# tohinz/multiple-objects-gan

Hardware: AMD Instinct MI355X
Metric: images/sec per G+D train step, 256x256 coco-attngan (higher is better)
Workload: dtype f32

## Files before the change

### include/mogan_hip.h

```cpp
#ifndef MOGAN_HIP_H
#define MOGAN_HIP_H

#include <stddef.h>
#include <stdint.h>

#ifdef __cplusplus
extern "C" {
#endif

typedef struct ihipStream_t* hipStream_t;

#define MOGAN_ERR_SHAPE (-1)
#define MOGAN_ERR_LAUNCH (-2)
#define MOGAN_ERR_WS (-3)

#define MOGAN_ACT_NONE 0
#define MOGAN_ACT_RELU 1
#define MOGAN_ACT_LRELU 2
#define MOGAN_ACT_GLU 3
#define MOGAN_ACT_TANH 4
#define MOGAN_ACT_SIGMOID 5

int mogan_abi_version(void);
int mogan_gemm_set_split_target(int blocks);
// ... 59 lines not shown
                          const int* dgrad, hipStream_t stream);
int mogan_conv2d_fwd_wp(const float* x, const float* w, const void* wprep, float* y, int B, int Cin, int Hs, int Ws, int Cout, int KH,
                        int KW, int stride, int ph, int pw, int up, void* ws, size_t ws_bytes, hipStream_t stream);
int mogan_conv2d_dgrad_wp(const float* dy, const float* w, const void* wprep, float* dx, int B, int Cin, int Hs, int Ws, int Cout,
                          int KH, int KW, int stride, int ph, int pw, int up, void* ws, size_t ws_bytes, hipStream_t stream);
int mogan_conv2d_wgrad(const float* dy, const float* x, float* dw, int B, int Cin, int Hs, int Ws, int Cout, int KH,
                       int KW, int stride, int ph, int pw, int up, int accumulate, void* ws, size_t ws_bytes,
                       hipStream_t stream);

int mogan_pk_conv_eligible(int B, int Cin, int Hs, int Ws, int Cout, int KH, int KW, int stride, int ph, int pw, int dgrad);
size_t mogan_pk_weight_bytes(int Cout, int Cin, int KH, int KW, int stride, int dgrad);
int mogan_pk_weight_pack(const float* w, void* wpk, int Cout, int Cin, int KH, int KW, int stride, int ph, int pw, int dgrad,
                         hipStream_t stream);
int mogan_pk_weight_pack_both(const float* w, void* wpk_fwd, void* wpk_dgrad, int Cout, int Cin, int KH, int KW, int stride, int ph,
                              int pw, hipStream_t stream);
int mogan_conv2d_fwd_pk(const float* x, const void* wpk, float* y, int B, int Cin, int Hs, int Ws, int Cout, int KH, int KW,
                        int stride, int ph, int pw, void* ws, size_t ws_bytes, hipStream_t stream);
int mogan_conv2d_dgrad_pk(const float* dy, const void* wpk, float* dx, int B, int Cin, int Hs, int Ws, int Cout, int KH, int KW,
                          int stride, int ph, int pw, void* ws, size_t ws_bytes, hipStream_t stream);
int mogan_pk_debug_force(int take_all, int cfg, int split);
int mogan_pk_wgrad_eligible(int B, int Cin, int Hs, int Ws, int Cout, int KH, int KW, int stride, int ph, int pw, size_t ws_bytes);
int mogan_conv2d_wgrad_pk(const float* dy, const float* x, float* dw, int B, int Cin, int Hs, int Ws, int Cout, int KH, int KW,
                          int stride, int ph, int pw, int accumulate, void* ws, size_t ws_bytes, hipStream_t stream);

size_t mogan_pk_panel_bytes(int B, int C, int HW);
int mogan_deep_block_eligible(int B, int Cin, int Hs, int Ws, int Cout, int KH, int KW, int stride, int ph, int pw, int act,
                              int groups);
int mogan_deep_conv_bn_act_fwd(const float* x, const void* xpanel, const void* wpk, const float* gamma, const float* beta,
                               float* rmean, float* rvar, float* y, float* stats, float* z, void* zpanel, int B, int Cin, int Hs,
                               int Ws, int Cout, int KH, int KW, int stride, int ph, int pw, float eps, float momentum, int act,
// ... 150 lines not shown
                         int s, int pad, hipStream_t stream);
int mogan_relu_bwd(const float* z, const float* dz, float* dx, long long n, int accumulate, hipStream_t stream);
int mogan_copy_strided(const float* src, long long src_bstride, float* dst, long long dst_bstride, int B, long long n,
                       hipStream_t stream);
int mogan_bilinear_fwd(const float* x, float* y, int planes, int H, int W, int OH, int OW, hipStream_t stream);
int mogan_bilinear_bwd(const float* dy, float* dx, int planes, int H, int W, int OH, int OW, hipStream_t stream);

int mogan_feed_crop_flip(const uint8_t* src, const int32_t* params, uint8_t* q, float* out, int B, int ori, int size,
                         hipStream_t stream);
int mogan_feed_resample(const uint8_t* in, uint8_t* tmp, float* out, const int32_t* bounds, const int32_t* kk, int ksize,
                        int B, int S, int OS, hipStream_t stream);

int mogan_adam_step(float* p, const float* g, float* m, float* v, float* ema, long long n, float lr, float beta1,
                    float beta2, float eps, int step, float* dev_state, int eps_mode, float grad_scale,
                    float ema_decay, hipStream_t stream);

int mogan_lstm_encoder_fwd(const long long* captions, const int* lens, const float* emb, const float* const* w_ih,
                           const float* const* w_hh, const float* const* b_ih, const float* const* b_hh, const float* h0,
                           const float* c0, float* words, float* sent, int B, int T, int Tmax, int V, int E, int H,
                           hipStream_t stream);

int mogan_lstm_encoder_train_fwd(const long long* captions, const int* lens, const float* emb, const float* const* w_ih,
                                 const float* const* w_hh, const float* const* b_ih, const float* const* b_hh, const float* h0,
                                 const float* c0, const uint8_t* keep_mask, float scale, float* words, float* sent, float* x,
                                 float* gates, float* cells, float* hprev, int B, int T, int Tmax, int V, int E, int H,
                                 hipStream_t stream);
int mogan_lstm_encoder_bwd(const float* dwords, const float* dsent, const int* lens, const float* gates, const float* cells,
                           const float* hprev, const float* c0, const float* const* w_hh, float* dgates, float* dbias, int B,
                           int Tmax, int H, hipStream_t stream);
int mogan_embedding_bwd(const long long* captions, const int* lens, const float* dx, const uint8_t* keep_mask, float scale,
// ... 66 lines not shown
```

### multiple-objects-gan_amd/attngan/trainer.py

```python
import dataclasses
import glob
import logging
import os
import time

import torch
import torch.distributed as dist

from ..hip import ops
from .evaluate import CheckpointEvaluation
from .miscc.config import cfg
from .miscc.losses import (KL_loss, discriminator_loss, discriminator_loss_fake, discriminator_loss_real,
                           generator_d_branch, generator_damsm_branch, generator_loss, generator_total, split_d_loss)
from .miscc.utils import copy_G_params, load_params, mkdir_p, weights_init
from .model_base import BNCallCounter
from .model import CNN_ENCODER, D_NET64, D_NET128, D_NET256, G_NET, RNN_ENCODER


class FlatAdam:

    ALIGN = 64

    def __init__(self, module, lr, with_ema=False, eps_mode=None):
        self.module, self.lr = module, float(lr)
# ... 5 lines not shown
            offs.append(total)
            total += (p.numel() + self.ALIGN - 1) // self.ALIGN * self.ALIGN
        self.offsets, self.numel = offs, total
        self.p = torch.zeros(total, dtype=torch.float32, device=dev)
        self.g = torch.zeros(total, dtype=torch.float32, device=dev)
        self.m = torch.zeros(total, dtype=torch.float32, device=dev)
        self.v = torch.zeros(total, dtype=torch.float32, device=dev)
        for p, o in zip(self.params, offs):
            self.p[o:o + p.numel()].copy_(p.data.reshape(-1))
            p.data = self.p[o:o + p.numel()].view_as(p)
            p.grad = self.g[o:o + p.numel()].view_as(p)
        self.ema = self.p.clone() if with_ema else None
        self.state = torch.zeros(3, dtype=torch.float32, device=dev)
        self._pk_cell = [0]
        self.packs = [ops.attach_packs(p, self._pk_cell) for p in self.params if p.dim() == 4] if dev.type == "cuda" else []
        self._hook = None
        if isinstance(module, torch.nn.Module):
            import weakref
            ref = weakref.ref(self)

            def _touch(m, keys, _ref=ref):
                me = _ref()
                if me is not None:
                    me.touch()
            self._hook = module.register_load_state_dict_post_hook(_touch)

    def close(self):
        if self._hook is not None:
            self._hook.remove()
            self._hook = None
        self.repack_on_touch = False
        self.packs = []

    repack_on_touch = False

    def touch(self):
        self._pk_cell[0] += 1
        if self.repack_on_touch:
            ops.repack_all(self.packs)

    def repack(self):
        self._pk_cell[0] += 1
        ops.repack_all(self.packs)

    on_zero = None

    def zero_grad(self):
        self.g.zero_()
        if self.on_zero is not None:
            self.on_zero()

    def step(self, grad_scale=1.0):
        ops.adam_step(self.p, self.g, self.m, self.v, self.ema, self.lr, 0.5, 0.999, 1e-8,
                      dev_state=self.state, eps_mode=self.eps_mode, grad_scale=grad_scale)
        self.repack()

    def ema_params(self):
        return [self.ema[o:o + p.numel()].view_as(p) for p, o in zip(self.params, self.offsets)]

    def state_dict(self):
        step = float(self.state[0].item())
        state = {i: {"step": torch.tensor(step), "exp_avg": self.m[o:o + p.numel()].view_as(p),
                     "exp_avg_sq": self.v[o:o + p.numel()].view_as(p)}
                 for i, (p, o) in enumerate(zip(self.params, self.offsets))}
        group = {"lr": self.lr, "betas": (0.5, 0.999), "eps": 1e-8, "weight_decay": 0, "amsgrad": False,
                 "params": list(range(len(self.params)))}
        return {"state": state, "param_groups": [group]}

    def load_state_dict(self, sd):
        if "state" in sd:
# ... 358 lines not shown
        return br.errD.clone(), br.g_loss.clone(), br.g_img


class TrainEngine:

    G_GRAPH_VARIANTS = 4

    def __init__(self, text_encoder, image_encoder, netG, netsD, distributed=False, use_graph=False, branch_graphs=None):
        self.text_encoder, self.image_encoder, self.netG, self.netsD = text_encoder, image_encoder, netG, netsD
        self.optG = FlatAdam(netG, cfg.TRAIN.GENERATOR_LR, with_ema=True)
        self.optDs = [FlatAdam(d, cfg.TRAIN.DISCRIMINATOR_LR) for d in netsD]
        self.bn_counter = BNCallCounter([netG] + list(netsD))
        self.distributed = bool(distributed) and dist.is_available() and dist.is_initialized() \
            and (dist.get_world_size() > 1 or bool(os.environ.get("MOGAN_FORCE_DIST")))
        self.world = dist.get_world_size() if self.distributed else 1
        self.use_graph = use_graph
        self._graph = None
        self._static = None
        self.last = {}
        self.graph_encoder = os.environ.get("MOGAN_GRAPH_ENCODER", "1") != "0" and not use_graph
        self._enc_graphs = {}
        self.multi_stream = os.environ.get("MOGAN_STREAMS", "1") != "0"
        if branch_graphs is None:
            branch_graphs = os.environ.get("MOGAN_BRANCH_GRAPHS", "1") != "0"
        if self.distributed and os.environ.get("MOGAN_BRANCH_GRAPHS_DP", "1") == "0":
            branch_graphs = False
        self.branch_graphs = bool(branch_graphs) and self.multi_stream and not use_graph
        gmode = os.environ.get("MOGAN_G_GRAPHS", "2")
        self.g_fwd_only = gmode == "2"
        self.g_graphs = self.branch_graphs and gmode != "0" and (self.g_fwd_only or not self.distributed)
# ... 764 lines not shown
```

### multiple-objects-gan_amd/csrc/mogan_elem.hip

```cpp
#include <hip/hip_runtime.h>
#include <stdint.h>
#include "../../include/mogan_hip.h"

namespace {

static inline int ok_launch() { return hipGetLastError() == hipSuccess ? 0 : MOGAN_ERR_LAUNCH; }

__global__ __launch_bounds__(256) void zero_fill_kernel(float* __restrict__ p, size_t n) {
    for (size_t i = (size_t)blockIdx.x * 256 + threadIdx.x; i < n; i += (size_t)gridDim.x * 256) p[i] = 0.f;
}
static inline void zero_fill(float* p, size_t n, hipStream_t st) {
    size_t b = (n + 255) / 256; if (b > 65536) b = 65536; if (b < 1) b = 1;
    hipLaunchKernelGGL(zero_fill_kernel, dim3((unsigned)b), dim3(256), 0, st, p, n);
}
#define POOL_LAUNCH(K, total, ...) do { if ((total) < (1ll << 31)) hipLaunchKernelGGL((K<unsigned>), __VA_ARGS__); \
                                         else hipLaunchKernelGGL((K<long long>), __VA_ARGS__); } while (0)
static inline unsigned nblk(long long n, int per = 256) {
    long long b = (n + per - 1) / per;
    return (unsigned)(b < 1 ? 1 : (b > 262144 ? 262144 : b));
}
__device__ __forceinline__ float sigmoidf_(float v) { return 1.f / (1.f + __expf(-v)); }

__device__ __forceinline__ float wave_sum(float v) {
#pragma unroll
// ... 349 lines not shown
                if (wy == 0.f) continue;
                float r = 0.f;
                for (int ox = xlo; ox <= xhi; ++ox) r += bil_w(ox, sw, W, x) * py[(size_t)oy * OW + ox];
                acc += wy * r;
            }
        }
        dx[i] = acc;
    }
}

__global__ __launch_bounds__(256) void adam_kernel(float* __restrict__ p, const float* __restrict__ g,
                                                   float* __restrict__ m, float* __restrict__ v, float* __restrict__ ema,
                                                   long long n4, long long n, float beta1, float beta2, float eps,
                                                   float step_size, float inv_sqrt_bc2, int eps_mode, float gscale,
                                                   float ema_decay, const float* __restrict__ dev_state) {
    if (dev_state) { step_size = dev_state[1]; inv_sqrt_bc2 = dev_state[2]; }
    for (long long i = (long long)blockIdx.x * 256 + threadIdx.x; i < n4; i += (long long)gridDim.x * 256) {
        const long long e = i * 4;
        float pv[4], gv[4], mv[4], vv[4], ev[4];
        const bool full = e + 3 < n;
        if (full) {
            *(float4*)pv = *(const float4*)(p + e); *(float4*)gv = *(const float4*)(g + e);
            *(float4*)mv = *(const float4*)(m + e); *(float4*)vv = *(const float4*)(v + e);
            if (ema) *(float4*)ev = *(const float4*)(ema + e);
        } else {
            for (int k = 0; k < 4; ++k) if (e + k < n) { pv[k] = p[e + k]; gv[k] = g[e + k]; mv[k] = m[e + k]; vv[k] = v[e + k]; if (ema) ev[k] = ema[e + k]; }
        }
#pragma unroll
        for (int k = 0; k < 4; ++k) {
            const float gg = gv[k] * gscale;
            mv[k] = mv[k] * beta1 + (1.f - beta1) * gg;
            vv[k] = vv[k] * beta2 + (1.f - beta2) * gg * gg;
            const float denom = eps_mode == 0 ? (sqrtf(vv[k]) * inv_sqrt_bc2 + eps) : (sqrtf(vv[k]) + eps);
            pv[k] = pv[k] - step_size * (mv[k] / denom);
            if (ema) ev[k] = ev[k] * ema_decay + (1.f - ema_decay) * pv[k];
        }
        if (full) {
            *(float4*)(p + e) = *(float4*)pv; *(float4*)(m + e) = *(float4*)mv; *(float4*)(v + e) = *(float4*)vv;
            if (ema) *(float4*)(ema + e) = *(float4*)ev;
        } else {
            for (int k = 0; k < 4; ++k) if (e + k < n) { p[e + k] = pv[k]; m[e + k] = mv[k]; v[e + k] = vv[k]; if (ema) ema[e + k] = ev[k]; }
        }
    }
}

__global__ __launch_bounds__(256) void reparam_fwd_kernel(const float* __restrict__ mu, const float* __restrict__ lv,
                                                          const float* __restrict__ eps, float* __restrict__ c, int n) {
    const int i = blockIdx.x * 256 + threadIdx.x;
    if (i < n) c[i] = eps[i] * __expf(0.5f * lv[i]) + mu[i];
}
// ... 377 lines not shown
int mogan_adam_step(float* p, const float* g, float* m, float* v, float* ema, long long n, float lr, float beta1,
                    float beta2, float eps, int step, float* dev_state, int eps_mode, float grad_scale,
                    float ema_decay, hipStream_t stream) {
    if (!p || !g || !m || !v || n <= 0 || (!dev_state && step < 1)) return MOGAN_ERR_SHAPE;
    if ((((uintptr_t)p | (uintptr_t)g | (uintptr_t)m | (uintptr_t)v | (uintptr_t)ema) & 15) != 0) return MOGAN_ERR_SHAPE;
    if (dev_state) { hipLaunchKernelGGL(adam_prep_kernel, dim3(1), dim3(1), 0, stream, dev_state, lr, beta1, beta2, eps_mode); step = 1; }
    const double bc1 = 1.0 - pow((double)beta1, (double)step), bc2 = 1.0 - pow((double)beta2, (double)step);
    const float step_size = eps_mode == 0 ? (float)(lr / bc1) : (float)(lr * sqrt(bc2) / bc1);
    const float inv_sqrt_bc2 = (float)(1.0 / sqrt(bc2));
    const long long n4 = (n + 3) / 4;
    hipLaunchKernelGGL(adam_kernel, dim3(nblk(n4)), dim3(256), 0, stream, p, g, m, v, ema, n4, n, beta1, beta2, eps,
                       step_size, inv_sqrt_bc2, eps_mode, grad_scale, ema_decay, (const float*)dev_state);
    return ok_launch();
}

}
```

### multiple-objects-gan_amd/csrc/mogan_pgemm.hip

```cpp
#include <hip/hip_runtime.h>
#include <stdint.h>
#include <stdlib.h>
#include <algorithm>
#include "../../include/mogan_hip.h"
#include "mogan_internal.h"
#include "mogan_mma.h"
#include "mogan_bn.h"
#include <type_traits>
#ifndef PK_NSET
#define PK_NSET 3
#endif
#define PK_TRIP (PK_NSET == 2 ? 2 : 6)

namespace {

typedef float f32x16 __attribute__((ext_vector_type(16)));

struct PkP {
    const unsigned char* A;
    const unsigned char* P;
    float* C; float* ws;
    int M, N, K;
    int Mt, KS;
    unsigned long long a_cls_stride;
// ... 288 lines not shown
            cls = py * p.s + px;
            ktap = (kh / p.s) * nkw + (kw / p.s);
        }
        const int ks = (ktap * p.Cc + c0) >> 4;
        unsigned char* d = p.A + (size_t)cls * p.cls_stride + ((size_t)blockIdx.x * p.KS + ks) * 3072 + lane * 16;
#pragma unroll
        for (int pl = 0; pl < 3; ++pl) *(uint4*)(d + pl * 1024) = make_uint4(w[pl][0], w[pl][1], w[pl][2], w[pl][3]);
    }
}


struct Wpack2P { const float* w; unsigned char* Af; unsigned char* Ad; int Cout, Cin, KW, s, ph, pw, KSf, KSd;
                 unsigned long long cls_stride; };

template <int KHW>
__global__ __launch_bounds__(256) void wpack2_kernel(const Wpack2P p) {
    __shared__ float L[KHW * 32 * 17];
    const int tid = threadIdx.x;
    const int co0 = blockIdx.x * 32, ci0 = blockIdx.y * 16;
    constexpr int ROW = 16 * KHW;
    if constexpr (ROW % 4 == 0) {
        for (int q = tid; q < 32 * ROW / 4; q += 256) {
            const int mi = q / (ROW / 4), r4 = (q - mi * (ROW / 4)) * 4;
            float4 v = make_float4(0.f, 0.f, 0.f, 0.f);
            if (co0 + mi < p.Cout) v = *(const float4*)(p.w + ((size_t)(co0 + mi) * p.Cin + ci0) * KHW + r4);
            const float e[4] = {v.x, v.y, v.z, v.w};
#pragma unroll
            for (int j = 0; j < 4; ++j) { const int r = r4 + j; L[((r % KHW) * 32 + mi) * 17 + r / KHW] = e[j]; }
        }
    } else {
        for (int q = tid; q < 32 * ROW; q += 256) {
            const int mi = q / ROW, r = q - mi * ROW;
            L[((r % KHW) * 32 + mi) * 17 + r / KHW] = (co0 + mi < p.Cout) ? p.w[((size_t)(co0 + mi) * p.Cin + ci0) * KHW + r] : 0.f;
        }
    }
    __syncthreads();
    const int nkw = p.KW / p.s;
    for (int it = tid; it < KHW * 128; it += 256) {
        const int tap = it >> 7, sub = it & 127;
        uint32_t w[3][4];
        unsigned char* d;
        if (sub < 64) {
            const int mi = sub & 31, h = sub >> 5;
            const float* v = &L[(tap * 32 + mi) * 17 + 8 * h];
#pragma unroll
            for (int j = 0; j < 4; ++j) x6_split2(v[2 * j], v[2 * j + 1], w[0][j], w[1][j], w[2][j]);
            const int ks = (tap * p.Cin + ci0) >> 4;
            d = p.Af + ((size_t)blockIdx.x * p.KSf + ks) * 3072 + sub * 16;
        } else {
            const int u = sub - 64, cil = u & 15, h = (u >> 4) & 1, kstep = u >> 5;
            const float* v = &L[(tap * 32 + kstep * 16 + h * 8) * 17 + cil];
#pragma unroll
            for (int j = 0; j < 4; ++j) x6_split2(v[(2 * j) * 17], v[(2 * j + 1) * 17], w[0][j], w[1][j], w[2][j]);
            const int kh = tap / p.KW, kw = tap - kh * p.KW;
            const int py = ((kh - p.ph) % p.s + p.s) % p.s, px = ((kw - p.pw) % p.s + p.s) % p.s;
            const int ktap = (kh / p.s) * nkw + (kw / p.s);
            const int ks = ((ktap * p.Cout + co0) >> 4) + kstep;
            const int ci = ci0 + cil, lane = (ci & 31) + 32 * h;
            d = p.Ad + (size_t)(py * p.s + px) * p.cls_stride + ((size_t)(ci >> 5) * p.KSd + ks) * 3072 + lane * 16;
            if (co0 + kstep * 16 >= p.Cout) continue;
        }
#pragma unroll
        for (int pl = 0; pl < 3; ++pl) *(uint4*)(d + pl * 1024) = make_uint4(w[pl][0], w[pl][1], w[pl][2], w[pl][3]);
    }
}


__global__ __launch_bounds__(256) void dypack_kernel(const float* __restrict__ dy, unsigned char* __restrict__ A, int Cout, int OHW,
                                                     int Npix, int KS) {
    const long long it = (long long)blockIdx.x * 256 + threadIdx.x;
    const int lane = (int)(it & 63);
    const long long u = it >> 6;
    const int ks = (int)(u % KS), mt = (int)(u / KS);
    const int co = mt * 32 + (lane & 31);
    const int n0 = ks * 16 + (lane >> 5) * 8;
    float v[8];
#pragma unroll
    for (int j = 0; j < 8; ++j) {
        const int n = n0 + j;
// ... 464 lines not shown
        return MOGAN_ERR_SHAPE;
    if (Cin % 32) return MOGAN_ERR_SHAPE;
    Wpack2P p{};
    p.w = w; p.Af = (unsigned char*)wpk_fwd; p.Ad = (unsigned char*)wpk_dgrad; p.Cout = Cout; p.Cin = Cin; p.KW = KW; p.s = stride;
    p.ph = ph; p.pw = pw; p.KSf = gf.KS; p.KSd = gd.KS; p.cls_stride = gd.cls_bytes;
    const dim3 grid((unsigned)cdiv(Cout, 32), (unsigned)(Cin / 16));
    switch (KH * KW) {
        case 16: hipLaunchKernelGGL(wpack2_kernel<16>, grid, dim3(256), 0, stream, p); break;
        case 9: hipLaunchKernelGGL(wpack2_kernel<9>, grid, dim3(256), 0, stream, p); break;
        case 1: hipLaunchKernelGGL(wpack2_kernel<1>, grid, dim3(256), 0, stream, p); break;
        default: {
            int rc = mogan_pk_weight_pack(w, wpk_fwd, Cout, Cin, KH, KW, stride, ph, pw, 0, stream);
            return rc ? rc : mogan_pk_weight_pack(w, wpk_dgrad, Cout, Cin, KH, KW, stride, ph, pw, 1, stream);
        }
    }
    return hipGetLastError() == hipSuccess ? 0 : MOGAN_ERR_LAUNCH;
}

static bool wgrad_pk_sizes(int B, int Cin, int Hs, int Ws, int Cout, int KH, int KW, int stride, int ph, int pw, int& OH, int& OW,
                           int& Kpad, long long& R, size_t& abytes, size_t& pbytes) {
    if (B <= 0 || Cin <= 0 || Cout <= 0 || Hs <= 0 || Ws <= 0 || KH <= 0 || KW <= 0 || stride <= 0) return false;
    OH = (Hs + 2 * ph - KH) / stride + 1; OW = (Ws + 2 * pw - KW) / stride + 1;
    if (OH <= 0 || OW <= 0) return false;
    const long long npix = (long long)B * OH * OW;
    if (npix > (1 << 20)) return false;
    Kpad = (int)((npix + 31) / 32 * 32);
    R = (long long)Cin * KH * KW;
    abytes = up256((size_t)((Cout + 31) / 32) * 32 * Kpad * 6);
    pbytes = up256((size_t)R * Kpad * 6);
    return pbytes < (1ull << 32) && (long long)Cout * R < (1ll << 31);
// ... 145 lines not shown
```

### multiple-objects-gan_amd/hip/lib.py

```python
import contextlib
import ctypes
import os

import torch

_HERE = os.path.dirname(os.path.dirname(os.path.abspath(__file__)))
LIB_PATH = os.environ.get("MOGAN_LIB") or os.path.join(_HERE, "libmogan_hip.so")

P, I, F, L, Z, D = ctypes.c_void_p, ctypes.c_int, ctypes.c_float, ctypes.c_longlong, ctypes.c_size_t, ctypes.c_double

SIGNATURES = {
    "mogan_abi_version": [],
    "mogan_gemm_set_split_target": [I],
    "mogan_stream_set_split_target": [P, I],
    "mogan_gemm_debug_force": [I, I],
    "mogan_gemm_group_min_tiles": [I],
    "mogan_mfma_form": [],
    "mogan_gemm_tune_set": [I, I, I, I, I, I, I],
    "mogan_gemm_tune_clear": [],
    "mogan_reserve_streams": [ctypes.c_int],
    "mogan_prof_enable": [I],
    "mogan_prof_collect": [P, I],
    "mogan_prof_dump": [ctypes.c_char_p],
    "mogan_conv2d_out_dims": [I, I, I, I, I, I, I, I, P, P],
# ... 3 lines not shown
    "mogan_conv2d_lrelu_fwd": [P, P, P] + [I] * 10 + [F, P, Z, P],
    "mogan_conv2d_affine_fwd": [P, P, P, P, P] + [I] * 11 + [P, Z, P],
    "mogan_affine_relu_bwd_out": [P, P, P, P, I, I, I, P],
    "mogan_conv2d_dgrad": [P, P, P] + [I] * 11 + [P, Z, P],
    "mogan_conv2d_wgrad": [P, P, P] + [I] * 12 + [P, Z, P],
    "mogan_wino_prep_bytes": [I] * 12,
    "mogan_wino_prep_group": [I, P, P, P, P, P, P],
    "mogan_conv_prep_bytes": [I] * 12,
    "mogan_conv_prep_group": [I, P, P, P, P, P, P, P],
    "mogan_conv2d_fwd_wp": [P, P, P, P] + [I] * 11 + [P, Z, P],
    "mogan_conv2d_dgrad_wp": [P, P, P, P] + [I] * 11 + [P, Z, P],
    "mogan_pk_conv_eligible": [I] * 11,
    "mogan_pk_weight_bytes": [I] * 6,
    "mogan_pk_weight_pack": [P, P] + [I] * 8 + [P],
    "mogan_pk_weight_pack_both": [P, P, P] + [I] * 7 + [P],
    "mogan_conv2d_fwd_pk": [P, P, P] + [I] * 10 + [P, Z, P],
    "mogan_conv2d_dgrad_pk": [P, P, P] + [I] * 10 + [P, Z, P],
    "mogan_pk_debug_force": [I, I, I],
    "mogan_pk_wgrad_eligible": [I] * 10 + [Z],
    "mogan_conv2d_wgrad_pk": [P, P, P] + [I] * 11 + [P, Z, P],
    "mogan_pk_panel_bytes": [I, I, I],
    "mogan_deep_block_eligible": [I] * 12,
    "mogan_deep_conv_bn_act_fwd": [P] * 11 + [I] * 10 + [F, F, I, F, I, P, Z, P],
    "mogan_deep_conv_bn_act_bwd": [P] * 9 + [I, P] + [I] * 10 + [I, F, I, P, Z, P],
    "mogan_upconv3x3_ws_bytes": [I, I],
    "mogan_upconv3x3_fwd": [P, P, P, I, I, I, I, I, P, Z, P],
    "mogan_lstm_encoder_fwd": [P] * 11 + [I] * 6 + [P],
    "mogan_upconv3x3_k4": [P, P, I, I, P],
    "mogan_upconv3x3_k4_group": [I, P, P, P, P, P],
    "mogan_upconv3x3_dgrad": [P, P, P, I, I, I, I, I, P, Z, P],
# ... 33 lines not shown
    "mogan_bce_fwd": [P, F, F, P, I, I, P],
    "mogan_bce_bwd": [P, F, F, P, P, I, P],
    "mogan_bce_logits_fwd": [P, F, F, P, I, I, P],
    "mogan_bce_logits_bwd": [P, F, F, P, P, I, P],
    "mogan_kl_fwd": [P, P, P, I, P],
    "mogan_kl_bwd": [P, P, P, P, P, I, P],
    "mogan_reparam_fwd": [P, P, P, P, I, P],
    "mogan_reparam_bwd": [P, P, P, P, P, I, P],
    "mogan_maxpool_fwd": [P, P, P, I, I, I, I, I, P],
    "mogan_maxpool_bwd": [P, P, P, I, I, I, I, I, P],
    "mogan_avgpool_fwd": [P, P, I, I, I, I, I, I, P],
    "mogan_avgpool_bwd": [P, P, I, I, I, I, I, I, P],
    "mogan_bilinear_fwd": [P, P, I, I, I, I, I, P],
    "mogan_bilinear_bwd": [P, P, I, I, I, I, I, P],
    "mogan_adam_step": [P, P, P, P, P, L, F, F, F, F, I, P, I, F, F, P],
    "mogan_conv2d_affine_fwd_ex": [P, L, P, P, P, P, L, P, L, I] + [I] * 11 + [P, Z, P],
    "mogan_conv2d_fwd_ex": [P, L, P, P, L, P, L, I] + [I] * 10 + [P, Z, P],
    "mogan_conv2d_dgrad_ex": [P, L, P, P, L, P, L, I] + [I] * 10 + [P, Z, P],
    "mogan_conv2d_affine_fwd_group": [I, P, P, Z, P],
    "mogan_conv2d_dgrad_group": [I, P, P, Z, P],
    "mogan_pk_group": [I, P, P],
    "mogan_panel_tail_group": [I, P, P],
    "mogan_maxpool_fwd_ex": [P, P, L, P, I, I, I, I, I, I, P],
    "mogan_maxpool_bwd_ex": [P, P, L, P, P, I, I, I, I, I, I, I, P],
    "mogan_avgpool_bwd_ex": [P, P, P, I, I, I, I, I, I, I, P],
    "mogan_copy_strided": [P, L, P, L, I, L, P],
    "mogan_relu_bwd": [P, P, P, L, I, P],
    "mogan_feed_crop_flip": [P, P, P, P, I, I, I, P],
    "mogan_feed_resample": [P, P, P, P, P, I, I, I, I, P],
    "mogan_damsm_words_fwd": [P, P, P, I, I, I, I, I, F, F, F, P, P, P, P, P, P],
# ... 200 lines not shown
```

### multiple-objects-gan_amd/hip/ops.py

```python
import contextlib
import ctypes
import os

import torch

from . import lib
from .lib import call, ptr, stream_ptr, workspace

ACT_NONE, ACT_RELU, ACT_LRELU, ACT_GLU, ACT_TANH, ACT_SIGMOID = 0, 1, 2, 3, 4, 5

ACT_TRACE = None


BN_DEFER = None


def bn_apply_deferred(pending):
    for mean, invstd, n, rm, rv, eps, momentum in pending:
        if rm is not None or rv is not None:
            call("mogan_bn_running_update", ptr(mean), ptr(invstd), ptr(rm), ptr(rv), mean.numel(), int(n), float(eps),
                 float(momentum), stream_ptr())
    del pending[:]


# ... 45 lines not shown
    def __init__(self):
        self.used, self.keep, self.parked = [], [], []


_wgrad_frames = [_WgradFrame()]


MERGE_WGRAD = os.environ.get("MOGAN_MERGE_WGRAD", "1") != "0"
_wgrad_pending = {}
MERGE_WGRAD_CAPTURED = True
_wgrad_ctx_depth = 0
_MERGE_K = 2048
_MERGE_W = 1 << 21


def _wgrad_launch(dy, x, w_shape, geom, g):
    stride, ph, pw, up = geom
    if WGRAD_SIDE_STREAM:
        cur, side = _wgrad_stream()
        side.wait_stream(cur)
        with torch.cuda.stream(side):
            conv2d_wgrad(dy, x, w_shape, stride, ph, pw, up, out=g, accumulate=True)
        fr = _wgrad_frames[-1]
        if side not in fr.used:
            fr.used.append(side)
        fr.keep.append((dy, x))
        _grad_hit(g, side)
    else:
        conv2d_wgrad(dy, x, w_shape, stride, ph, pw, up, out=g, accumulate=True)
        _grad_hit(g)


def _wgrad_accumulate(dy, x, w, geom, g):
    K = dy.shape[0] * dy.shape[2] * dy.shape[3]
    if not (MERGE_WGRAD and _wgrad_ctx_depth > 0 and K <= _MERGE_K and w.numel() >= _MERGE_W) \
            or (torch.cuda.is_current_stream_capturing() and not MERGE_WGRAD_CAPTURED):
        _wgrad_launch(dy, x, w.shape, geom, g)
        return
    cur = torch.cuda.current_stream()
    key = (g.data_ptr(), cur.cuda_stream)
    prev = _wgrad_pending.pop(key, None)
    if prev is None:
        _wgrad_pending[key] = (dy, x, tuple(w.shape), geom, g, cur)
        _wgrad_frames[-1].parked.append(key)
# ... 181 lines not shown
        self.slots = {}
        self.elig = {}
        self.wino = {}
        self.wbytes = {}
        self.k4 = None
        self.k4pk = None

    def _pack(self, dgrad, slot):
        Cout, Cin, KH, KW = self.w.shape
        st = stream_ptr()
        stride, ph, pw = slot.geom
        call("mogan_pk_weight_pack", ptr(self.w), slot.buf.data_ptr(), Cout, Cin, KH, KW, stride, ph, pw, dgrad, st)
        _stamp(st, [(slot, self.cell)])
        PK_STATS["packs"] += 1

    def repack(self):
        s0, s1 = self.slots.get(0), self.slots.get(1)
        Cout, Cin, KH, KW = self.w.shape
        if s0 is not None and s1 is not None and s0.geom == s1.geom and Cin % 32 == 0 and Cout % 32 == 0:
            stride, ph, pw = s0.geom
            st = stream_ptr()
            call("mogan_pk_weight_pack_both", ptr(self.w), s0.buf.data_ptr(), s1.buf.data_ptr(), Cout, Cin, KH, KW, stride, ph, pw, st)
            _stamp(st, [(s0, self.cell), (s1, self.cell)])
            PK_STATS["packs"] += 1
            return
        for dgrad, slot in self.slots.items():
            self._pack(dgrad, slot)

    def pointer(self, dgrad, B, Hs, Ws, stride, ph, pw):
        key = (dgrad, B, Hs, Ws, stride, ph, pw)
        e = self.elig.get(key)
        Cout, Cin, KH, KW = self.w.shape
        if e is None:
            e = self.elig[key] = bool(lib.load().mogan_pk_conv_eligible(B, Cin, Hs, Ws, Cout, KH, KW, stride, ph, pw, dgrad))
# ... 64 lines not shown
    PK_STATS["wino_preps"] = PK_STATS.get("wino_preps", 0) + 1


def k4_build_group(pks):
    n = len(pks)
    if not n:
        return
    ws = [[pk.w.data_ptr() for pk in pks], [pk.k4.buf.data_ptr() for pk in pks]]
    shapes = [pk.w.shape for pk in pks]
    st = stream_ptr()
    call("mogan_upconv3x3_k4_group", n, *_group_args(n, ws, [[s[i] for s in shapes] for i in (0, 1)]), st)
    _stamp(st, [(pk.k4, pk.cell) for pk in pks])
    PK_STATS["k4_builds"] = PK_STATS.get("k4_builds", 0) + 1


def repack_all(packs):
    items, k4s = [], []
    for pk in packs:
        pk.repack()
        items += [(pk, d, im) for d, im in pk.wino.items()]
        if pk.k4 is not None:
            k4s.append(pk)
            items += [(pk.k4pk, d, im) for d, im in pk.k4pk.wino.items()]
    k4_build_group(k4s)
    wino_prep(items)


def _wino_prep_ptr(w, dgrad, B, Hs, Ws, stride, ph, pw, up):
    pk = getattr(w, "_mogan_pk", None)
    if pk is None or not WINO_PREP:
        return None
    return pk.wino_pointer(dgrad, B, Hs, Ws, stride, ph, pw, up)


# ... 1611 lines not shown

def avg_pool2d(x, k, s=None, pad=0):
    return PoolFn.apply(x, "avg", k, s or k, pad, 0, 0)


def bilinear_resize(x, OH, OW):
    return PoolFn.apply(x, "bilinear", 0, 0, 0, OH, OW)


def adam_step(p, g, m, v, ema, lr, beta1, beta2, eps, step=0, dev_state=None, eps_mode=0, grad_scale=1.0,
              ema_decay=0.999):
    call("mogan_adam_step", ptr(p), ptr(g), ptr(m), ptr(v), ptr(ema), p.numel(), lr, beta1, beta2, eps, step,
         ptr(dev_state), eps_mode, grad_scale, ema_decay, stream_ptr())


def _rnn_encoder_args(captions, lens, emb_weight, rnn, states):
    cell = "lstm" if isinstance(rnn, torch.nn.LSTM) else "gru" if isinstance(rnn, torch.nn.GRU) else None
    if (cell is None or len(states) != (2 if cell == "lstm" else 1) or rnn.num_layers != 1 or not rnn.bidirectional
            or not rnn.batch_first or rnn.hidden_size != 128 or not rnn.bias or getattr(rnn, "proj_size", 0)):
        return None
    H = rnn.hidden_size
    if captions.dim() != 2 or emb_weight.dim() != 2:
        return None
    B, T = captions.shape
    V, E = emb_weight.shape
    lens = [int(v) for v in lens]
    Tmax = max(lens) if lens else 0
    if (len(lens) != B or B > 64 or Tmax < 1 or Tmax > 32 or Tmax > T or E > 320 or E % 4 or min(lens) < 0
            or captions.dtype != torch.int64 or rnn.input_size != E):
        return None
# ... 129 lines not shown
```

Measured before the change: 461.0.

## Fuse discriminator Adam update with weight packing and overwrite first wgrad

Adds a kernel that applies the Adam update to each 4-D conv weight tile and writes the packed forward and dgrad layouts in the same pass, so the separate Adam sweep and the repack re-read of weights are merged. Non-conv parameter ranges are updated by a separate apply kernel after a one-thread prep kernel computes the bias-correction coefficients on device. It also skips zeroing those fused gradient slices: the first wgrad of each round overwrites instead of accumulating, tracked by a round counter keyed on the gradient pointer. Enabled by default for discriminator optimizers when not distributed. The pointer-keyed bookkeeping adds complexity and a risk of stale or missed gradients.

```diff
diff --git a/include/mogan_hip.h b/include/mogan_hip.h
--- a/include/mogan_hip.h
+++ b/include/mogan_hip.h
@@ -97,6 +97,10 @@
                          hipStream_t stream);
 int mogan_pk_weight_pack_both(const float* w, void* wpk_fwd, void* wpk_dgrad, int Cout, int Cin, int KH, int KW, int stride, int ph,
                               int pw, hipStream_t stream);
+int mogan_pk_adam_pack_both(float* p, float* g, float* m, float* v, float* ema, void* wpk_fwd, void* wpk_dgrad, int Cout, int Cin,
+                            int KH, int KW, int stride, int ph, int pw, float lr, float beta1, float beta2, float eps, int step,
+                            const float* dev_state, int eps_mode, float grad_scale, float ema_decay, int zero_g,
+                            hipStream_t stream);
 int mogan_conv2d_fwd_pk(const float* x, const void* wpk, float* y, int B, int Cin, int Hs, int Ws, int Cout, int KH, int KW,
                         int stride, int ph, int pw, void* ws, size_t ws_bytes, hipStream_t stream);
 int mogan_conv2d_dgrad_pk(const float* dy, const void* wpk, float* dx, int B, int Cin, int Hs, int Ws, int Cout, int KH, int KW,
@@ -277,6 +281,9 @@
 int mogan_adam_step(float* p, const float* g, float* m, float* v, float* ema, long long n, float lr, float beta1,
                     float beta2, float eps, int step, float* dev_state, int eps_mode, float grad_scale,
                     float ema_decay, hipStream_t stream);
+int mogan_adam_prep(float* dev_state, float lr, float beta1, float beta2, int eps_mode, hipStream_t stream);
+int mogan_adam_apply(float* p, const float* g, float* m, float* v, float* ema, long long n, float beta1, float beta2, float eps,
+                     const float* dev_state, int eps_mode, float grad_scale, float ema_decay, hipStream_t stream);
 
 int mogan_lstm_encoder_fwd(const long long* captions, const int* lens, const float* emb, const float* const* w_ih,
                            const float* const* w_hh, const float* const* b_ih, const float* const* b_hh, const float* h0,
diff --git a/multiple-objects-gan_amd/attngan/trainer.py b/multiple-objects-gan_amd/attngan/trainer.py
--- a/multiple-objects-gan_amd/attngan/trainer.py
+++ b/multiple-objects-gan_amd/attngan/trainer.py
@@ -43,6 +43,10 @@
         self.state = torch.zeros(3, dtype=torch.float32, device=dev)
         self._pk_cell = [0]
         self.packs = [ops.attach_packs(p, self._pk_cell) for p in self.params if p.dim() == 4] if dev.type == "cuda" else []
+        self._pk_range = {id(p._mogan_pk): (o, p.numel()) for p, o in zip(self.params, offs) if p.dim() == 4} if self.packs else {}
+        self._fused, self._rest, self._round, self._ow_ptrs = [], [(0, total)], [0], []
+        import weakref
+        weakref.finalize(self, ops.overwrite_drop, self._ow_ptrs)
         self._hook = None
         if isinstance(module, torch.nn.Module):
             import weakref
@@ -60,6 +64,7 @@
             self._hook = None
         self.repack_on_touch = False
         self.packs = []
+        self._unfuse()
 
     repack_on_touch = False
 
@@ -75,14 +80,60 @@
     on_zero = None
 
     def zero_grad(self):
-        self.g.zero_()
+        self._round[0] += 1
+        if not self._fused:
+            self.g.zero_()
+        else:
+            for a, b in self._rest:
+                self.g[a:b].zero_()
         if self.on_zero is not None:
             self.on_zero()
 
+    fuse_packs = False
+
+    def _unfuse(self):
+        ops.overwrite_drop(self._ow_ptrs)
+        self._fused, self._rest = [], [(0, self.numel)]
+
     def step(self, grad_scale=1.0):
-        ops.adam_step(self.p, self.g, self.m, self.v, self.ema, self.lr, 0.5, 0.999, 1e-8,
-                      dev_state=self.state, eps_mode=self.eps_mode, grad_scale=grad_scale)
-        self.repack()
+        take = self.fuse_packs and ops.DIRECT_GRAD and not ops.GRAD_HOOKS
+        fused = [pk for pk in self.packs if pk.adam_fusable()] if take else []
+        overwrite = bool(ops.WGRAD_OVERWRITE)
+        if self._ow_ptrs:
+            for o, n in self._fused:
+                if ops.overwrite_stale(self.g[o:o + n]):
+                    self.g[o:o + n].zero_()
+            if not fused or not overwrite:
+                ops.overwrite_drop(self._ow_ptrs)
+        if not fused:
+            self._unfuse()
+            ops.adam_step(self.p, self.g, self.m, self.v, self.ema, self.lr, 0.5, 0.999, 1e-8,
+                          dev_state=self.state, eps_mode=self.eps_mode, grad_scale=grad_scale)
+            self.repack()
+            return
+        ranges = sorted(self._pk_range[id(pk)] for pk in fused)
+        kw = dict(dev_state=self.state, eps_mode=self.eps_mode, grad_scale=grad_scale)
+        sl = lambda t, o, n: None if t is None else t[o:o + n]
+        ops.adam_prep(self.state, self.lr, 0.5, 0.999, self.eps_mode)
+        st = ops.stream_ptr()
+        for pk in fused:
+            o, n = self._pk_range[id(pk)]
+            g = self.g[o:o + n]
+            if overwrite and ops.overwrite_register(g, self._round):
+                self._ow_ptrs.append(g.data_ptr())
+            ops.adam_pack_both(pk, self.p[o:o + n], g, self.m[o:o + n], self.v[o:o + n], sl(self.ema, o, n), self.lr, 0.5, 0.999,
+                               1e-8, zero_g=not overwrite, **kw)
+        rest, at = [], 0
+        for o, n in ranges + [(self.numel, 0)]:
+            if o > at:
+                rest.append((at, o))
+            at = o + n
+        for a, b in rest:
+            ops.adam_apply(self.p[a:b], self.g[a:b], self.m[a:b], self.v[a:b], sl(self.ema, a, b - a), 0.5, 0.999, 1e-8, **kw)
+        self._fused, self._rest = ranges, rest
+        self._pk_cell[0] += 1
+        ops._stamp(st, [(pk.slots[d], pk.cell) for pk in fused for d in (0, 1)])
+        ops.repack_all(self.packs, packed={id(pk) for pk in fused})
 
     def ema_params(self):
         return [self.ema[o:o + p.numel()].view_as(p) for p, o in zip(self.params, self.offsets)]
@@ -471,6 +522,8 @@
         self.distributed = bool(distributed) and dist.is_available() and dist.is_initialized() \
             and (dist.get_world_size() > 1 or bool(os.environ.get("MOGAN_FORCE_DIST")))
         self.world = dist.get_world_size() if self.distributed else 1
+        for o in self.optDs:
+            o.fuse_packs = ops.FUSE_ADAM_PACK and not self.distributed
         self.use_graph = use_graph
         self._graph = None
         self._static = None
diff --git a/multiple-objects-gan_amd/csrc/mogan_adam.h b/multiple-objects-gan_amd/csrc/mogan_adam.h
--- /dev/null
+++ b/multiple-objects-gan_amd/csrc/mogan_adam.h
@@ -0,0 +1,27 @@
+#ifndef MOGAN_ADAM_H
+#define MOGAN_ADAM_H
+#include <hip/hip_runtime.h>
+
+struct AdamCoef { float beta1, beta2, eps, step_size, inv_sqrt_bc2, gscale, ema_decay; int eps_mode; };
+
+__device__ __forceinline__ AdamCoef adam_coef(float beta1, float beta2, float eps, float step_size, float inv_sqrt_bc2,
+                                              int eps_mode, float gscale, float ema_decay,
+                                              const float* __restrict__ dev_state) {
+    AdamCoef k;
+    if (dev_state) { step_size = dev_state[1]; inv_sqrt_bc2 = dev_state[2]; }
+    k.beta1 = beta1; k.beta2 = beta2; k.eps = eps; k.step_size = step_size; k.inv_sqrt_bc2 = inv_sqrt_bc2;
+    k.gscale = gscale; k.ema_decay = ema_decay; k.eps_mode = eps_mode;
+    return k;
+}
+
+template <bool HAS_EMA>
+__device__ __forceinline__ void adam_update(const AdamCoef& k, float& p, float g, float& m, float& v, float& e) {
+    const float gg = g * k.gscale;
+    m = m * k.beta1 + (1.f - k.beta1) * gg;
+    v = v * k.beta2 + (1.f - k.beta2) * gg * gg;
+    const float denom = k.eps_mode == 0 ? (sqrtf(v) * k.inv_sqrt_bc2 + k.eps) : (sqrtf(v) + k.eps);
+    p = p - k.step_size * (m / denom);
+    if (HAS_EMA) e = e * k.ema_decay + (1.f - k.ema_decay) * p;
+}
+
+#endif
diff --git a/multiple-objects-gan_amd/csrc/mogan_elem.hip b/multiple-objects-gan_amd/csrc/mogan_elem.hip
--- a/multiple-objects-gan_amd/csrc/mogan_elem.hip
+++ b/multiple-objects-gan_amd/csrc/mogan_elem.hip
@@ -1,6 +1,7 @@
 #include <hip/hip_runtime.h>
 #include <stdint.h>
 #include "../../include/mogan_hip.h"
+#include "mogan_adam.h"
 
 namespace {
 
@@ -387,7 +388,7 @@
                                                    long long n4, long long n, float beta1, float beta2, float eps,
                                                    float step_size, float inv_sqrt_bc2, int eps_mode, float gscale,
                                                    float ema_decay, const float* __restrict__ dev_state) {
-    if (dev_state) { step_size = dev_state[1]; inv_sqrt_bc2 = dev_state[2]; }
+    const AdamCoef ac = adam_coef(beta1, beta2, eps, step_size, inv_sqrt_bc2, eps_mode, gscale, ema_decay, dev_state);
     for (long long i = (long long)blockIdx.x * 256 + threadIdx.x; i < n4; i += (long long)gridDim.x * 256) {
         const long long e = i * 4;
         float pv[4], gv[4], mv[4], vv[4], ev[4];
@@ -401,12 +402,8 @@
         }
 #pragma unroll
         for (int k = 0; k < 4; ++k) {
-            const float gg = gv[k] * gscale;
-            mv[k] = mv[k] * beta1 + (1.f - beta1) * gg;
-            vv[k] = vv[k] * beta2 + (1.f - beta2) * gg * gg;
-            const float denom = eps_mode == 0 ? (sqrtf(vv[k]) * inv_sqrt_bc2 + eps) : (sqrtf(vv[k]) + eps);
-            pv[k] = pv[k] - step_size * (mv[k] / denom);
-            if (ema) ev[k] = ev[k] * ema_decay + (1.f - ema_decay) * pv[k];
+            if (ema) adam_update<true>(ac, pv[k], gv[k], mv[k], vv[k], ev[k]);
+            else adam_update<false>(ac, pv[k], gv[k], mv[k], vv[k], ev[k]);
         }
         if (full) {
             *(float4*)(p + e) = *(float4*)pv; *(float4*)(m + e) = *(float4*)mv; *(float4*)(v + e) = *(float4*)vv;
@@ -814,4 +811,19 @@
     return ok_launch();
 }
 
-}
+int mogan_adam_prep(float* dev_state, float lr, float beta1, float beta2, int eps_mode, hipStream_t stream) {
+    if (!dev_state) return MOGAN_ERR_SHAPE;
+    hipLaunchKernelGGL(adam_prep_kernel, dim3(1), dim3(1), 0, stream, dev_state, lr, beta1, beta2, eps_mode);
+    return ok_launch();
+}
+int mogan_adam_apply(float* p, const float* g, float* m, float* v, float* ema, long long n, float beta1, float beta2, float eps,
+                     const float* dev_state, int eps_mode, float grad_scale, float ema_decay, hipStream_t stream) {
+    if (!p || !g || !m || !v || !dev_state || n <= 0) return MOGAN_ERR_SHAPE;
+    if ((((uintptr_t)p | (uintptr_t)g | (uintptr_t)m | (uintptr_t)v | (uintptr_t)ema) & 15) != 0) return MOGAN_ERR_SHAPE;
+    const long long n4 = (n + 3) / 4;
+    hipLaunchKernelGGL(adam_kernel, dim3(nblk(n4)), dim3(256), 0, stream, p, g, m, v, ema, n4, n, beta1, beta2, eps, 0.f, 0.f,
+                       eps_mode, grad_scale, ema_decay, dev_state);
+    return ok_launch();
+}
+
+}
diff --git a/multiple-objects-gan_amd/csrc/mogan_pgemm.hip b/multiple-objects-gan_amd/csrc/mogan_pgemm.hip
--- a/multiple-objects-gan_amd/csrc/mogan_pgemm.hip
+++ b/multiple-objects-gan_amd/csrc/mogan_pgemm.hip
@@ -6,6 +6,8 @@
 #include "mogan_internal.h"
 #include "mogan_mma.h"
 #include "mogan_bn.h"
+#include "mogan_adam.h"
+#include <math.h>
 #include <type_traits>
 #ifndef PK_NSET
 #define PK_NSET 3
@@ -326,6 +328,38 @@
                  unsigned long long cls_stride; };
 
 template <int KHW>
+__device__ __forceinline__ void wpack2_store(const float* L, const Wpack2P& p, int tid, int co0, int ci0) {
+    const int nkw = p.KW / p.s;
+    for (int it = tid; it < KHW * 128; it += 256) {
+        const int tap = it >> 7, sub = it & 127;
+        uint32_t w[3][4];
+        unsigned char* d;
+        if (sub < 64) {
+            const int mi = sub & 31, h = sub >> 5;
+            const float* v = &L[(tap * 32 + mi) * 17 + 8 * h];
+#pragma unroll
+            for (int j = 0; j < 4; ++j) x6_split2(v[2 * j], v[2 * j + 1], w[0][j], w[1][j], w[2][j]);
+            const int ks = (tap * p.Cin + ci0) >> 4;
+            d = p.Af + ((size_t)blockIdx.x * p.KSf + ks) * 3072 + sub * 16;
+        } else {
+            const int u = sub - 64, cil = u & 15, h = (u >> 4) & 1, kstep = u >> 5;
+            const float* v = &L[(tap * 32 + kstep * 16 + h * 8) * 17 + cil];
+#pragma unroll
+            for (int j = 0; j < 4; ++j) x6_split2(v[(2 * j) * 17], v[(2 * j + 1) * 17], w[0][j], w[1][j], w[2][j]);
+            const int kh = tap / p.KW, kw = tap - kh * p.KW;
+            const int py = ((kh - p.ph) % p.s + p.s) % p.s, px = ((kw - p.pw) % p.s + p.s) % p.s;
+            const int ktap = (kh / p.s) * nkw + (kw / p.s);
+            const int ks = ((ktap * p.Cout + co0) >> 4) + kstep;
+            const int ci = ci0 + cil, lane = (ci & 31) + 32 * h;
+            d = p.Ad + (size_t)(py * p.s + px) * p.cls_stride + ((size_t)(ci >> 5) * p.KSd + ks) * 3072 + lane * 16;
+            if (co0 + kstep * 16 >= p.Cout) continue;
+        }
+#pragma unroll
+        for (int pl = 0; pl < 3; ++pl) *(uint4*)(d + pl * 1024) = make_uint4(w[pl][0], w[pl][1], w[pl][2], w[pl][3]);
+    }
+}
+
+template <int KHW>
 __global__ __launch_bounds__(256) void wpack2_kernel(const Wpack2P p) {
     __shared__ float L[KHW * 32 * 17];
     const int tid = threadIdx.x;
@@ -347,34 +381,42 @@
         }
     }
     __syncthreads();
-    const int nkw = p.KW / p.s;
-    for (int it = tid; it < KHW * 128; it += 256) {
-        const int tap = it >> 7, sub = it & 127;
-        uint32_t w[3][4];
-        unsigned char* d;
-        if (sub < 64) {
-            const int mi = sub & 31, h = sub >> 5;
-            const float* v = &L[(tap * 32 + mi) * 17 + 8 * h];
-#pragma unroll
-            for (int j = 0; j < 4; ++j) x6_split2(v[2 * j], v[2 * j + 1], w[0][j], w[1][j], w[2][j]);
-            const int ks = (tap * p.Cin + ci0) >> 4;
-            d = p.Af + ((size_t)blockIdx.x * p.KSf + ks) * 3072 + sub * 16;
-        } else {
-            const int u = sub - 64, cil = u & 15, h = (u >> 4) & 1, kstep = u >> 5;
-            const float* v = &L[(tap * 32 + kstep * 16 + h * 8) * 17 + cil];
-#pragma unroll
-            for (int j = 0; j < 4; ++j) x6_split2(v[(2 * j) * 17], v[(2 * j + 1) * 17], w[0][j], w[1][j], w[2][j]);
-            const int kh = tap / p.KW, kw = tap - kh * p.KW;
-            const int py = ((kh - p.ph) % p.s + p.s) % p.s, px = ((kw - p.pw) % p.s + p.s) % p.s;
-            const int ktap = (kh / p.s) * nkw + (kw / p.s);
-            const int ks = ((ktap * p.Cout + co0) >> 4) + kstep;
-            const int ci = ci0 + cil, lane = (ci & 31) + 32 * h;
-            d = p.Ad + (size_t)(py * p.s + px) * p.cls_stride + ((size_t)(ci >> 5) * p.KSd + ks) * 3072 + lane * 16;
-            if (co0 + kstep * 16 >= p.Cout) continue;
-        }
-#pragma unroll
-        for (int pl = 0; pl < 3; ++pl) *(uint4*)(d + pl * 1024) = make_uint4(w[pl][0], w[pl][1], w[pl][2], w[pl][3]);
-    }
+    wpack2_store<KHW>(L, p, tid, co0, ci0);
+}
+
+struct Wpack2AdamP { Wpack2P pk; float* p; float* g; float* m; float* v; float* ema; const float* dev_state;
+                     float beta1, beta2, eps, step_size, inv_sqrt_bc2, gscale, ema_decay; int eps_mode, zero_g; };
+
+template <int KHW, bool HAS_EMA>
+__global__ __launch_bounds__(256) void wpack2_adam_kernel(const Wpack2AdamP a) {
+    __shared__ float L[KHW * 32 * 17];
+    const Wpack2P& p = a.pk;
+    const int tid = threadIdx.x;
+    const int co0 = blockIdx.x * 32, ci0 = blockIdx.y * 16;
+    constexpr int ROW = 16 * KHW;
+    static_assert(ROW % 4 == 0, "16-byte accesses of a co row");
+    const AdamCoef k = adam_coef(a.beta1, a.beta2, a.eps, a.step_size, a.inv_sqrt_bc2, a.eps_mode, a.gscale, a.ema_decay,
+                                 a.dev_state);
+    for (int q = tid; q < 32 * ROW / 4; q += 256) {
+        const int mi = q / (ROW / 4), r4 = (q - mi * (ROW / 4)) * 4;
+        float pv[4] = {0.f, 0.f, 0.f, 0.f};
+        if (co0 + mi < p.Cout) {
+            const size_t o = ((size_t)(co0 + mi) * p.Cin + ci0) * KHW + r4;
+            float gv[4], mv[4], vv[4], ev[4] = {0.f, 0.f, 0.f, 0.f};
+            *(float4*)pv = *(const float4*)(a.p + o); *(float4*)gv = *(const float4*)(a.g + o);
+            *(float4*)mv = *(const float4*)(a.m + o); *(float4*)vv = *(const float4*)(a.v + o);
+            if (HAS_EMA) *(float4*)ev = *(const float4*)(a.ema + o);
+#pragma unroll
+            for (int j = 0; j < 4; ++j) adam_update<HAS_EMA>(k, pv[j], gv[j], mv[j], vv[j], ev[j]);
+            *(float4*)(a.p + o) = *(float4*)pv; *(float4*)(a.m + o) = *(float4*)mv; *(float4*)(a.v + o) = *(float4*)vv;
+            if (HAS_EMA) *(float4*)(a.ema + o) = *(float4*)ev;
+            if (a.zero_g) *(float4*)(a.g + o) = make_float4(0.f, 0.f, 0.f, 0.f);
+        }
+#pragma unroll
+        for (int j = 0; j < 4; ++j) { const int r = r4 + j; L[((r % KHW) * 32 + mi) * 17 + r / KHW] = pv[j]; }
+    }
+    __syncthreads();
+    wpack2_store<KHW>(L, p, tid, co0, ci0);
 }
 
 
@@ -869,6 +911,42 @@
             return rc ? rc : mogan_pk_weight_pack(w, wpk_dgrad, Cout, Cin, KH, KW, stride, ph, pw, 1, stream);
         }
     }
+    return hipGetLastError() == hipSuccess ? 0 : MOGAN_ERR_LAUNCH;
+}
+
+int mogan_pk_adam_pack_both(float* p, float* g, float* m, float* v, float* ema, void* wpk_fwd, void* wpk_dgrad, int Cout, int Cin,
+                            int KH, int KW, int stride, int ph, int pw, float lr, float beta1, float beta2, float eps, int step,
+                            const float* dev_state, int eps_mode, float grad_scale, float ema_decay, int zero_g,
+                            hipStream_t stream) {
+    PkGeom gf, gd;
+    if (!p || !g || !m || !v || !wpk_fwd || !wpk_dgrad || (!dev_state && step < 1)) return MOGAN_ERR_SHAPE;
+    if ((((uintptr_t)p | (uintptr_t)g | (uintptr_t)m | (uintptr_t)v | (uintptr_t)ema | (uintptr_t)wpk_fwd | (uintptr_t)wpk_dgrad) & 15) != 0)
+        return MOGAN_ERR_SHAPE;
+    if (!pk_geom(Cout, Cin, KH, KW, stride, 0, gf) || !pk_geom(Cout, Cin, KH, KW, stride, 1, gd)) return MOGAN_ERR_SHAPE;
+    if (Cin % 32 || Cout % 32) return MOGAN_ERR_SHAPE;
+    const int taps = KH * KW;
+    if (taps != 16 && taps != 9 && taps != 1) return MOGAN_ERR_SHAPE;
+    Wpack2AdamP a{};
+    a.pk.w = p; a.pk.Af = (unsigned char*)wpk_fwd; a.pk.Ad = (unsigned char*)wpk_dgrad; a.pk.Cout = Cout; a.pk.Cin = Cin;
+    a.pk.KW = KW; a.pk.s = stride; a.pk.ph = ph; a.pk.pw = pw; a.pk.KSf = gf.KS; a.pk.KSd = gd.KS; a.pk.cls_stride = gd.cls_bytes;
+    a.p = p; a.g = g; a.m = m; a.v = v; a.ema = ema; a.dev_state = dev_state;
+    a.beta1 = beta1; a.beta2 = beta2; a.eps = eps; a.eps_mode = eps_mode; a.gscale = grad_scale; a.ema_decay = ema_decay;
+    a.zero_g = zero_g ? 1 : 0;
+    if (!dev_state) {
+        const double bc1 = 1.0 - pow((double)beta1, (double)step), bc2 = 1.0 - pow((double)beta2, (double)step);
+        a.step_size = eps_mode == 0 ? (float)(lr / bc1) : (float)(lr * sqrt(bc2) / bc1);
+        a.inv_sqrt_bc2 = (float)(1.0 / sqrt(bc2));
+    }
+    const dim3 grid((unsigned)(Cout / 32), (unsigned)(Cin / 16));
+#define MOGAN_ADAM_PACK(T)                                                                                          \
+    if (ema) hipLaunchKernelGGL((wpack2_adam_kernel<T, true>), grid, dim3(256), 0, stream, a);                      \
+    else hipLaunchKernelGGL((wpack2_adam_kernel<T, false>), grid, dim3(256), 0, stream, a)
+    switch (taps) {
+        case 16: MOGAN_ADAM_PACK(16); break;
+        case 9: MOGAN_ADAM_PACK(9); break;
+        default: MOGAN_ADAM_PACK(1); break;
+    }
+#undef MOGAN_ADAM_PACK
     return hipGetLastError() == hipSuccess ? 0 : MOGAN_ERR_LAUNCH;
 }
 
diff --git a/multiple-objects-gan_amd/hip/lib.py b/multiple-objects-gan_amd/hip/lib.py
--- a/multiple-objects-gan_amd/hip/lib.py
+++ b/multiple-objects-gan_amd/hip/lib.py
@@ -41,6 +41,7 @@
     "mogan_pk_weight_bytes": [I] * 6,
     "mogan_pk_weight_pack": [P, P] + [I] * 8 + [P],
     "mogan_pk_weight_pack_both": [P, P, P] + [I] * 7 + [P],
+    "mogan_pk_adam_pack_both": [P] * 7 + [I] * 7 + [F, F, F, F, I, P, I, F, F, I, P],
     "mogan_conv2d_fwd_pk": [P, P, P] + [I] * 10 + [P, Z, P],
     "mogan_conv2d_dgrad_pk": [P, P, P] + [I] * 10 + [P, Z, P],
     "mogan_pk_debug_force": [I, I, I],
@@ -104,6 +105,8 @@
     "mogan_bilinear_fwd": [P, P, I, I, I, I, I, P],
     "mogan_bilinear_bwd": [P, P, I, I, I, I, I, P],
     "mogan_adam_step": [P, P, P, P, P, L, F, F, F, F, I, P, I, F, F, P],
+    "mogan_adam_prep": [P, F, F, F, I, P],
+    "mogan_adam_apply": [P, P, P, P, P, L, F, F, F, P, I, F, F, P],
     "mogan_conv2d_affine_fwd_ex": [P, L, P, P, P, P, L, P, L, I] + [I] * 11 + [P, Z, P],
     "mogan_conv2d_fwd_ex": [P, L, P, P, L, P, L, I] + [I] * 10 + [P, Z, P],
     "mogan_conv2d_dgrad_ex": [P, L, P, P, L, P, L, I] + [I] * 10 + [P, Z, P],
diff --git a/multiple-objects-gan_amd/hip/ops.py b/multiple-objects-gan_amd/hip/ops.py
--- a/multiple-objects-gan_amd/hip/ops.py
+++ b/multiple-objects-gan_amd/hip/ops.py
@@ -83,20 +83,53 @@
 _MERGE_W = 1 << 21
 
 
+FUSE_ADAM_PACK = os.environ.get("MOGAN_FUSE_ADAM_PACK", "1") != "0"
+WGRAD_OVERWRITE = os.environ.get("MOGAN_WGRAD_OVERWRITE", "1") != "0"
+_OVERWRITE = {}
+
+
+def overwrite_register(g, round_cell):
+    if g.data_ptr() in _OVERWRITE:
+        return False
+    _OVERWRITE[g.data_ptr()] = [round_cell, round_cell[0]]
+    return True
+
+
+def overwrite_drop(ptrs):
+    for p in ptrs:
+        _OVERWRITE.pop(p, None)
+    del ptrs[:]
+
+
+def overwrite_stale(g):
+    rec = _OVERWRITE.get(g.data_ptr())
+    return rec is not None and rec[1] != rec[0][0]
+
+
+def _first_of_round(g):
+    rec = _OVERWRITE.get(g.data_ptr()) if _OVERWRITE else None
+    if rec is None:
+        return False
+    first = rec[1] != rec[0][0]
+    rec[1] = rec[0][0]
+    return first
+
+
 def _wgrad_launch(dy, x, w_shape, geom, g):
     stride, ph, pw, up = geom
+    acc = not _first_of_round(g)
     if WGRAD_SIDE_STREAM:
         cur, side = _wgrad_stream()
         side.wait_stream(cur)
         with torch.cuda.stream(side):
-            conv2d_wgrad(dy, x, w_shape, stride, ph, pw, up, out=g, accumulate=True)
+            conv2d_wgrad(dy, x, w_shape, stride, ph, pw, up, out=g, accumulate=acc)
         fr = _wgrad_frames[-1]
         if side not in fr.used:
             fr.used.append(side)
         fr.keep.append((dy, x))
         _grad_hit(g, side)
     else:
-        conv2d_wgrad(dy, x, w_shape, stride, ph, pw, up, out=g, accumulate=True)
+        conv2d_wgrad(dy, x, w_shape, stride, ph, pw, up, out=g, accumulate=acc)
         _grad_hit(g)
 
 
@@ -308,10 +341,18 @@
         _stamp(st, [(slot, self.cell)])
         PK_STATS["packs"] += 1
 
+    def both_in_use(self):
+        s0, s1 = self.slots.get(0), self.slots.get(1)
+        Cout, Cin = self.w.shape[:2]
+        return s0 is not None and s1 is not None and s0.geom == s1.geom and Cin % 32 == 0 and Cout % 32 == 0
+
+    def adam_fusable(self):
+        return self.both_in_use() and self.w.shape[2] * self.w.shape[3] in (16, 9, 1)
+
     def repack(self):
         s0, s1 = self.slots.get(0), self.slots.get(1)
         Cout, Cin, KH, KW = self.w.shape
-        if s0 is not None and s1 is not None and s0.geom == s1.geom and Cin % 32 == 0 and Cout % 32 == 0:
+        if self.both_in_use():
             stride, ph, pw = s0.geom
             st = stream_ptr()
             call("mogan_pk_weight_pack_both", ptr(self.w), s0.buf.data_ptr(), s1.buf.data_ptr(), Cout, Cin, KH, KW, stride, ph, pw, st)
@@ -406,10 +447,11 @@
     PK_STATS["k4_builds"] = PK_STATS.get("k4_builds", 0) + 1
 
 
-def repack_all(packs):
+def repack_all(packs, packed=()):
     items, k4s = [], []
     for pk in packs:
-        pk.repack()
+        if id(pk) not in packed:
+            pk.repack()
         items += [(pk, d, im) for d, im in pk.wino.items()]
         if pk.k4 is not None:
             k4s.append(pk)
@@ -2051,6 +2093,26 @@
          ptr(dev_state), eps_mode, grad_scale, ema_decay, stream_ptr())
 
 
+def adam_prep(dev_state, lr, beta1, beta2, eps_mode=0):
+    call("mogan_adam_prep", ptr(dev_state), lr, beta1, beta2, eps_mode, stream_ptr())
+
+
+def adam_apply(p, g, m, v, ema, beta1, beta2, eps, dev_state, eps_mode=0, grad_scale=1.0, ema_decay=0.999):
+    call("mogan_adam_apply", ptr(p), ptr(g), ptr(m), ptr(v), ptr(ema), p.numel(), beta1, beta2, eps, ptr(dev_state), eps_mode,
+         grad_scale, ema_decay, stream_ptr())
+
+
+def adam_pack_both(pk, p, g, m, v, ema, lr, beta1, beta2, eps, step=0, dev_state=None, eps_mode=0, grad_scale=1.0,
+                   ema_decay=0.999, zero_g=True):
+    Cout, Cin, KH, KW = pk.w.shape
+    s0, s1 = pk.slots[0], pk.slots[1]
+    stride, ph, pw = s0.geom
+    call("mogan_pk_adam_pack_both", ptr(p), ptr(g), ptr(m), ptr(v), ptr(ema), s0.buf.data_ptr(), s1.buf.data_ptr(), Cout, Cin, KH,
+         KW, stride, ph, pw, lr, beta1, beta2, eps, step, ptr(dev_state), eps_mode, grad_scale, ema_decay, 1 if zero_g else 0,
+         stream_ptr())
+    PK_STATS["adam_packs"] = PK_STATS.get("adam_packs", 0) + 1
+
+
 def _rnn_encoder_args(captions, lens, emb_weight, rnn, states):
     cell = "lstm" if isinstance(rnn, torch.nn.LSTM) else "gru" if isinstance(rnn, torch.nn.GRU) else None
     if (cell is None or len(states) != (2 if cell == "lstm" else 1) or rnn.num_layers != 1 or not rnn.bidirectional
```

After: 468.1 (median of 6 runs). +1.5%, better.
